# segasai/rvspecfit

Measured on AMD Instinct MI355X. Metric: spectra/sec (CCF+chi2 grid) DESI 3-arm, higher is better.
Workload: dtype f64

## Files before the change

### rvspecfit_amd/csrc/ccf_fft.hip

```cpp
#include "common.h"

#define XC_NT 512
#define XC_NTW(n2) ((n2) >> 3)

struct XcLds {
  int t1;
  int c0;
  int t1c;
  int ca;
  size_t bytes;
};
#define XW_NT1C 73
#define XC_LDS_MAX (159 * 1024)
__host__ __device__ constexpr XcLds xc_lds_pair(int n2, int nlag) {
  const int t1 = n2, c0 = t1 + XC_NTW(n2);
  return {t1, c0, 0, 0, sizeof(double2) * (size_t)c0 + sizeof(double) * 2 * (size_t)nlag};
}
__host__ __device__ constexpr XcLds xc_lds_ws(int n2, int nlag, bool ratio) {
  const int t1 = 2 * n2, c0 = t1 + XC_NTW(n2), t1c = c0 + ((nlag + 1) >> 1),
            ca = t1c + XW_NT1C;
  return {t1, c0, t1c, ca,
          sizeof(double2) * (size_t)ca + (ratio ? sizeof(double) * (size_t)nlag : 0)};
}
__host__ __device__ constexpr XcLds xc_lds_ws2(int n2, int nlag) {
  const int t1 = 4 * n2, c0 = t1 + XC_NTW(n2);
  return {t1, c0, 0, 0, sizeof(double2) * (size_t)c0 + sizeof(double) * 2 * (size_t)nlag};
}
__host__ __device__ constexpr bool xc_lds_fits(const XcLds &L, int n2, int nimg,
                                               int nrow, int nlag, bool ws, bool ratio) {
  const size_t D2 = sizeof(double2), D = sizeof(double);
  size_t end = D2 * (size_t)nimg * n2;
  if (D2 * L.t1 < end) return false;
  end = D2 * (L.t1 + XC_NTW(n2));
  if (D2 * L.c0 < end) return false;
  end = D2 * L.c0 + D * (size_t)nrow * nlag;
  if (ws) {
    if (D2 * L.t1c < end) return false;
    end = D2 * (L.t1c + 72);
    if (D2 * L.ca < end) return false;
    end = D2 * L.ca + (ratio ? D * (size_t)nlag : 0);
  }
  return end <= L.bytes && L.bytes <= XC_LDS_MAX;
}
constexpr bool xc_lds_check() {
  for (int nlag = 2; nlag <= 512; nlag++)
    for (int n2 = 2048; n2 <= 4096; n2 *= 2) {
      for (int ratio = 0; ratio < 2; ratio++)
        if (!xc_lds_fits(xc_lds_ws(n2, nlag, ratio), n2, 2, 1, nlag, true, ratio))
          return false;
      if (n2 == 2048 && !xc_lds_fits(xc_lds_ws2(n2, nlag), n2, 4, 2, nlag, false, false))
        return false;
      if (!xc_lds_fits(xc_lds_pair(n2, nlag), n2, 1, 2, nlag, false, false))
        return false;
    }
  return true;
}
static_assert(xc_lds_check(), "an LDS array of a cross-correlation kernel overlaps "
                              "its neighbour or ends beyond the launch's request");

__device__ __forceinline__ double2 cmul(double2 a, double2 b) {
  return make_double2(a.x * b.x - a.y * b.y, a.x * b.y + a.y * b.x);
}
__device__ __forceinline__ double2 cadd(double2 a, double2 b) {
  return make_double2(a.x + b.x, a.y + b.y);
}
__device__ __forceinline__ double2 csub(double2 a, double2 b) {
  return make_double2(a.x - b.x, a.y - b.y);
}
template <int SIGN>
__device__ __forceinline__ double2 cmuli(double2 a) {
  return (SIGN > 0) ? make_double2(-a.y, a.x) : make_double2(a.y, -a.x);
}

__host__ __device__ inline int xc_plan(int log2n, int *rad) {
  int n = 0, l = log2n;
  while (l >= 3) {
    rad[n++] = 8;
    l -= 3;
  }
  if (l == 2) rad[n++] = 4;
  if (l == 1) rad[n++] = 2;
  return n;
}

extern "C" int rvs_ccf_fft_pos(int nfft, int f) {
  int log2n = 0;
  while ((2 << log2n) < nfft) log2n++;
  int rad[8];
  const int np = xc_plan(log2n, rad);
  int n2 = nfft >> 1, pos = 0, m = n2;
  for (int p = 0; p < np; p++) {
    const int q = f % rad[p];
    f /= rad[p];
    m /= rad[p];
    pos += q * m;
  }
  return pos;
}

template <int SIGN>
__device__ __forceinline__ void dft4(double2 &a0, double2 &a1, double2 &a2,
                                     double2 &a3) {
  const double2 t0 = cadd(a0, a2), t1 = csub(a0, a2);
  const double2 t2 = cadd(a1, a3), t3 = cmuli<SIGN>(csub(a1, a3));
  a0 = cadd(t0, t2);
  a2 = csub(t0, t2);
  a1 = cadd(t1, t3);
  a3 = csub(t1, t3);
}

template <int SIGN>
__device__ __forceinline__ void dft8(double2 *a) {
  double2 e0 = a[0], e1 = a[2], e2 = a[4], e3 = a[6];
  double2 o0 = a[1], o1 = a[3], o2 = a[5], o3 = a[7];
  dft4<SIGN>(e0, e1, e2, e3);
  dft4<SIGN>(o0, o1, o2, o3);
  const double h = 0.70710678118654752440;
  const double2 w1o = (SIGN > 0) ? make_double2(h * (o1.x - o1.y), h * (o1.x + o1.y))
                                 : make_double2(h * (o1.x + o1.y), h * (o1.y - o1.x));
  const double2 w2o = cmuli<SIGN>(o2);
  const double2 w3o = (SIGN > 0) ? make_double2(-h * (o3.x + o3.y), h * (o3.x - o3.y))
                                 : make_double2(h * (o3.y - o3.x), -h * (o3.x + o3.y));
  a[0] = cadd(e0, o0);
  a[4] = csub(e0, o0);
  a[1] = cadd(e1, w1o);
  a[5] = csub(e1, w1o);
  a[2] = cadd(e2, w2o);
  a[6] = csub(e2, w2o);
  a[3] = cadd(e3, w3o);
  a[7] = csub(e3, w3o);
}

template <int SIGN>
__device__ __forceinline__ double2 twid(const double2 *__restrict__ tw, int e,
                                        int nfft) {
  const int half = nfft >> 1;
  double2 w = (e < half) ? tw[e] : tw[e - half];
  if (e >= half) {
    w.x = -w.x;
    w.y = -w.y;
  }
  if (SIGN < 0) w.y = -w.y;
  return w;
}

#ifdef RVS_XC_TIMING
__device__ unsigned long long xc_dbg[16];
#define XC_T(i)                                        \
  do {                                                 \
    __syncthreads();                                   \
    if (threadIdx.x == 0) {                            \
      const unsigned long long t_ = wall_clock64();    \
      atomicAdd(&xc_dbg[i], t_ - t_prev);              \
      t_prev = t_;                                     \
    }                                                  \
  } while (0)
extern "C" int rvs_dbg_read_xc(unsigned long long *out) {
  return hipMemcpyFromSymbol(out, HIP_SYMBOL(xc_dbg), sizeof(xc_dbg)) ==
                 hipSuccess
             ? 0
             : -1;
}
#else
#define XC_T(i)
#endif

template <int NT>
__device__ __forceinline__ void xc_fill_twiddles(double2 *a, int n2,
                                                 const double2 *__restrict__ tw) {
  const int ntw = XC_NTW(n2);
  if ((ntw & 63) == 0) {
    const int lane = threadIdx.x & 63;
    for (int i0 = (threadIdx.x >> 6) * 64; i0 < ntw; i0 += NT) {
      __builtin_amdgcn_global_load_lds(
          (const __attribute__((address_space(1))) void *)(tw + 2 * (i0 + lane)),
          (__attribute__((address_space(3))) void *)(a + n2 + i0), 16, 0, 0);
    }
    return;
  }
  for (int i = threadIdx.x; i < ntw; i += NT) a[n2 + i] = tw[2 * i];
}

struct XcMasks {
  unsigned g, b0, b7;
};
template <int NT>
__device__ __forceinline__ XcMasks xc_load_masks(const uint8_t *__restrict__ prune,
                                                 int n2) {
  XcMasks m = {0u, 0u, 0u};
  if (prune && (n2 >> 3) <= NT) {
    const int t = threadIdx.x, B = t >> 3;
    if (t < (n2 >> 3)) m.g = prune[(n2 >> 6) + t];
    if (B < (n2 >> 6)) {
      m.b0 = prune[(n2 >> 6) + 8 * B];
      m.b7 = prune[(n2 >> 6) + 8 * B + 7];
    }
  }
  return m;
}

template <int SIGN, int NT>
__device__ void fft_lds(double2 *a, int log2n, const double2 *__restrict__ tw,
                        const uint8_t *__restrict__ prune = nullptr,
                        const XcMasks *pm = nullptr) {
  const int n2 = 1 << log2n, nfft = n2 << 1;
  const double2 *T1 = a + n2;
  auto tw1 = [&](int r, int tws) -> double2 {
    double2 w = T1[r << (tws - 1)];
    if (SIGN < 0) w.y = -w.y;
    return w;
  };
  int rad[8];
  const int np = xc_plan(log2n, rad);
  const bool pr = prune && np >= 2 && rad[np - 1] == 8 && rad[np - 2] == 8;
  bool fold = false;
  const bool can_fold = pr && pm && (n2 >> 3) <= NT;
  int lgM = log2n;
  for (int p = 0; p < np; p++) {
    if (can_fold && p == 0) {
      const int pos8 = threadIdx.x & 7;
      const unsigned m = pm->g;
      const bool bad =
          m != 0 && !((pos8 == 0 && m == 0x01u) || (pos8 == 7 && m == 0x80u));
      fold = !__syncthreads_or(bad);
    }
    if (fold && p == np - 2) {
      __syncthreads();
      const int s = threadIdx.x & 7;
      for (int B = threadIdx.x >> 3; B < (n2 >> 6); B += NT >> 3) {
        const unsigned m0 = pm->b0 & 1u, m63 = pm->b7 >> 7;
        if (!(m0 | m63)) continue;
        double2 v[8];
#pragma unroll
        for (int j = 0; j < 8; j++) v[j] = a[B * 64 + s + 8 * j];
        dft8<SIGN>(v);
        double2 w = T1[s << (log2n - 6)];
        if (SIGN > 0) w.y = -w.y;
        double2 x63 = cmul(v[7], w), x0 = v[0];
        auto sum8 = [](double x) {
          x += dpp_get<0xb1, 0xf, 0xf>(x);
          x += dpp_get<0x4e, 0xf, 0xf>(x);
          x += dpp_get<0x141, 0xf, 0xf>(x);
          return x;
        };
        if (m0) {
          x0.x = sum8(x0.x);
          x0.y = sum8(x0.y);
          if (s == 0) a[B * 64] = x0;
        }
        if (m63) {
          x63.x = sum8(x63.x);
          x63.y = sum8(x63.y);
          if (s == 0) a[B * 64 + 63] = x63;
        }
      }
      break;
    }
    const int R = rad[p], lgR = (R == 8) ? 3 : (R == 4 ? 2 : 1);
    const int lgMp = lgM - lgR, Mp = 1 << lgMp;
    const int tws = log2n + 1 - lgM;
    if (!(can_fold && p == 0)) __syncthreads();
    for (int u = threadIdx.x; u < (n2 >> lgR); u += NT) {
      const int blk = u >> lgMp, r = u & (Mp - 1);
      const int base = (blk << lgM) + r;
      if (pr && p == np - 2) {
        const unsigned mask = prune[blk];
        if (mask == 0) continue;
        double2 v[8];
#pragma unroll
        for (int j = 0; j < 8; j++) v[j] = a[base + Mp * j];
        dft8<SIGN>(v);
        double2 wp[8];
        wp[0] = make_double2(1.0, 0.0);
        wp[1] = tw1(r, tws);
        wp[2] = cmul(wp[1], wp[1]);
        wp[3] = cmul(wp[2], wp[1]);
        wp[4] = cmul(wp[2], wp[2]);
        wp[7] = cmul(wp[4], wp[3]);
        wp[5] = cmul(wp[4], wp[1]);
        wp[6] = cmul(wp[4], wp[2]);
#pragma unroll
        for (int q = 0; q < 8; q++)
          if (mask & (1u << q))
            a[base + Mp * q] = (q == 0) ? v[0] : cmul(v[q], wp[q]);
        continue;
      }
      if (pr && p == np - 1) {
        const unsigned mask = prune[(n2 >> 6) + u];
        if (mask == 0) continue;
        double2 v[8];
#pragma unroll
        for (int j = 0; j < 8; j++) v[j] = a[base + j];
        dft8<SIGN>(v);
#pragma unroll
        for (int q = 0; q < 8; q++)
          if (mask & (1u << q)) a[base + q] = v[q];
        continue;
      }
      if (R == 8) {
        double2 v[8];
#pragma unroll
        for (int j = 0; j < 8; j++) v[j] = a[base + Mp * j];
        dft8<SIGN>(v);
        if (Mp > 1) {
          const double2 w1 = tw1(r, tws);
          v[1] = cmul(v[1], w1);
          const double2 w2 = cmul(w1, w1);
          v[2] = cmul(v[2], w2);
          double2 wc = cmul(w2, w1);
          v[3] = cmul(v[3], wc);
          const double2 w4 = cmul(w2, w2);
          v[4] = cmul(v[4], w4);
          v[7] = cmul(v[7], cmul(w4, wc));
          wc = cmul(w4, w1);
          v[5] = cmul(v[5], wc);
          v[6] = cmul(v[6], cmul(w4, w2));
        }
#pragma unroll
        for (int q = 0; q < 8; q++) a[base + Mp * q] = v[q];
      } else if (R == 4) {
        double2 v0 = a[base], v1 = a[base + Mp],
                v2 = a[base + 2 * Mp], v3 = a[base + 3 * Mp];
        dft4<SIGN>(v0, v1, v2, v3);
        if (Mp > 1) {
          const double2 w1 = twid<SIGN>(tw, r << tws, nfft);
          const double2 w2 = cmul(w1, w1), w3 = cmul(w2, w1);
          v1 = cmul(v1, w1);
          v2 = cmul(v2, w2);
          v3 = cmul(v3, w3);
        }
        a[base] = v0;
        a[base + Mp] = v1;
        a[base + 2 * Mp] = v2;
        a[base + 3 * Mp] = v3;
      } else {
        const double2 v0 = a[base], v1 = a[base + Mp];
        double2 d = csub(v0, v1);
        if (Mp > 1) d = cmul(d, twid<SIGN>(tw, r << tws, nfft));
        a[base] = cadd(v0, v1);
        a[base + Mp] = d;
      }
    }
    lgM = lgMp;
  }
  __syncthreads();
}

__device__ __forceinline__ int fft_pos(int f, int log2n) {
  int pos = 0, lgm = log2n;
  while (lgm > 0) {
    const int lgr = lgm >= 3 ? 3 : lgm;
    lgm -= lgr;
    pos += (f & ((1 << lgr) - 1)) << lgm;
    f >>= lgr;
  }
  return pos;
}

template <bool MODEL>
__global__ void __launch_bounds__(XC_NT)
    ccf_rfft_kernel(const double *__restrict__ proc_spec,
                    const double *__restrict__ proc_ivar, int nfft, int log2n,
                    const double2 *__restrict__ tw, double2 *__restrict__ work,
                    double2 *__restrict__ work2) {
  extern __shared__ double2 fa[];
  const int b = blockIdx.x, which = blockIdx.y, tid = threadIdx.x;
  const int n2 = nfft >> 1;
  const double *ps = proc_spec + (int64_t)b * nfft;
  const double *pi = MODEL ? nullptr : proc_ivar + (int64_t)b * nfft;
  xc_fill_twiddles<XC_NT>(fa, n2, tw);
  for (int n = tid; n < n2; n += XC_NT) {
    double x0, x1;
    if (MODEL) {
      x0 = ps[2 * n];
      x1 = ps[2 * n + 1];
      if (which) {
        x0 *= x0;
        x1 *= x1;
      }
    } else if (which == 0) {
      x0 = ps[2 * n] * pi[2 * n];
      x1 = ps[2 * n + 1] * pi[2 * n + 1];
    } else {
      x0 = pi[2 * n];
      x1 = pi[2 * n + 1];
    }
    fa[n] = make_double2(x0, x1);
  }
  fft_lds<-1, XC_NT>(fa, log2n, tw);
  double2 *out = MODEL ? (which ? work2 : work) + (int64_t)b * (n2 + 1)
                       : work + ((int64_t)b * 2 + which) * (n2 + 1);
  for (int k = tid; k <= n2; k += XC_NT) {
    double2 X;
    if (k == 0 || k == n2) {
      const double2 z0 = fa[0];
      X = make_double2(k == 0 ? z0.x + z0.y : z0.x - z0.y, 0.0);
    } else {
      const double2 zk = fa[fft_pos(k, log2n)];
      const double2 zm = fa[fft_pos(n2 - k, log2n)];
      const double2 e = make_double2(zk.x + zm.x, zk.y - zm.y);
      const double2 d = make_double2(zk.x - zm.x, zk.y + zm.y);
      const double2 q = cmul(twid<-1>(tw, k, nfft), d);
      X = make_double2(0.5 * (e.x + q.y), 0.5 * (e.y - q.x));
    }
    out[k] = MODEL ? X : make_double2(X.x, -X.y);
  }
}

int ccf_model_rfft(const double *model, int nfft, int M, const double *twid,
                   double *fft, double *fft2, hipStream_t st) {
  int log2n = 0;
  while ((2 << log2n) < nfft) log2n++;
  if ((2 << log2n) != nfft || nfft < 64 || nfft > 16384 || M < 1) return RVS_E_ARG;
  static bool attr_set = false;
  if (!attr_set) {
    (void)hipFuncSetAttribute((const void *)ccf_rfft_kernel<true>,
                              hipFuncAttributeMaxDynamicSharedMemorySize, XC_LDS_MAX);
    (void)hipGetLastError();
    attr_set = true;
  }
  for (int b0 = 0; b0 < M; b0 += 65535) {
    const int nb = (M - b0 < 65535) ? (M - b0) : 65535;
    const int64_t o = (int64_t)b0 * ((nfft >> 1) + 1);
    hipLaunchKernelGGL(ccf_rfft_kernel<true>, dim3(nb, 2), dim3(XC_NT),
                       xc_lds_pair(nfft >> 1, 0).bytes, st,
                       model + (int64_t)b0 * nfft, (const double *)nullptr, nfft, log2n,
                       reinterpret_cast<const double2 *>(twid),
                       reinterpret_cast<double2 *>(fft) + o,
                       reinterpret_cast<double2 *>(fft2) + o);
    RVS_LAUNCH_CHECK();
  }
  return 0;
}

#define XB_NT 512

__device__ __forceinline__ bool xc_job(unsigned bid, int T, int B, int G, int &b,
                                       int &t) {
  const int xcd = bid & 7;
  const int slot = bid >> 3;
  const int tt = slot % G;
  const int q = slot / G;
  b = q % B;
  const int g = q / B;
  t = xcd + 8 * (g * G + tt);
  return t < T;
}
__host__ inline int64_t xc_nblocks(int T, int B, int G) {
  const int ntx = (T + 7) >> 3;
  const int ngrp = (ntx + G - 1) / G;
  return 8ll * ngrp * G * B;
}
__host__ inline int xc_group(int T, int nfft) {
  const int64_t per_t = 2ll * ((nfft >> 1) + 1) * 16;
  if (per_t * T <= (16ll << 20)) return 0;
#ifndef XC_GROUP_BYTES
#define XC_GROUP_BYTES (2ll << 20)
#endif
  int G = (int)(XC_GROUP_BYTES / per_t);
  const int ntx = (T + 7) >> 3;
  if (G < 1) G = 1;
  if (G > ntx) G = ntx;
  return G;
}

__global__ void __launch_bounds__(XB_NT)
    __attribute__((amdgpu_waves_per_eu(4, 4)))
    ccf_xcorr_kernel(const double2 *__restrict__ work, int nfft, int log2n,
                     const double2 *__restrict__ tfft,
                     const double2 *__restrict__ tfft2, int T,
                     const double2 *__restrict__ tw, int continuum,
                     const int32_t *__restrict__ lag_pos,
                     const double *__restrict__ lag_vel, int nlag,
                     const int32_t *__restrict__ ilo,
                     const double *__restrict__ vgrid, int nvel, double beta,
                     const uint8_t *__restrict__ prune,
                     double *__restrict__ chisq, int B, int G) {
  extern __shared__ double2 fa[];
  const int n2 = nfft >> 1, npair = n2 >> 1;
  double *c0 = reinterpret_cast<double *>(fa + xc_lds_pair(n2, nlag).c0);
  double *c1 = c0 + nlag;
  int t = blockIdx.x, b = blockIdx.y;
  if (G > 0 && !xc_job(blockIdx.x, T, B, G, b, t)) return;
  const int tid = threadIdx.x;
  const double2 *Sc = work + ((int64_t)b * 2) * (n2 + 1);
  const double2 *Vc = Sc + (n2 + 1);
  const double2 *F = tfft + (int64_t)t * (n2 + 1);
  const double2 *F2 = tfft2 + (int64_t)t * (n2 + 1);
  const double inv_n = 1.0 / nfft;
  const int npass = continuum ? 1 : 2;
  xc_fill_twiddles<XB_NT>(fa, n2, tw);
  XcMasks pmask = xc_load_masks<XB_NT>(prune, n2);
#ifdef RVS_XC_TIMING
  unsigned long long t_prev = wall_clock64();
#endif
  double *out = chisq + ((int64_t)b * T + t) * nvel;
  const bool pre = (nlag <= XB_NT) && (nvel <= XB_NT);
  int pre_pos = 0, pre_lo = 0;
  double pre_x0 = 0, pre_x1 = 1, pre_xg = 0, pre_old = 0;
  if (pre) {
    const int tv = min(tid, nvel - 1);
    pre_pos = lag_pos[min(tid, nlag - 1)];
    pre_lo = ilo[tv];
    pre_xg = vgrid[tv];
    pre_old = out[tv];
  }
  for (int pass = 0; pass < npass; pass++) {
    if (continuum) {
      typedef int v4i_t __attribute__((ext_vector_type(4)));
      const int nbytes = (n2 + 1) * 16;
      const __amdgpu_buffer_rsrc_t rF = __builtin_amdgcn_make_buffer_rsrc(
          (void *)F, 0, nbytes, 0x00020000);
      const __amdgpu_buffer_rsrc_t rF2 = __builtin_amdgcn_make_buffer_rsrc(
          (void *)F2, 0, nbytes, 0x00020000);
      const __amdgpu_buffer_rsrc_t rS = __builtin_amdgcn_make_buffer_rsrc(
          (void *)Sc, 0, nbytes, 0x00020000);
      const __amdgpu_buffer_rsrc_t rV = __builtin_amdgcn_make_buffer_rsrc(
          (void *)Vc, 0, nbytes, 0x00020000);
      const __amdgpu_buffer_rsrc_t rT = __builtin_amdgcn_make_buffer_rsrc(
          (void *)tw, 0, (npair + 1) * 16, 0x00020000);
      auto ld = [](const __amdgpu_buffer_rsrc_t &r, int off) {
        const v4i_t v = __builtin_amdgcn_raw_buffer_load_b128(r, off, 0, 0);
        return make_double2(__hiloint2double(v.y, v.x),
                            __hiloint2double(v.w, v.z));
      };
      if (tid == 0) {
        const double2 p1 = cmul(F[0], Sc[0]), p2 = cmul(F2[0], Vc[0]);
        const double2 q1 = cmul(F[n2], Sc[n2]), q2 = cmul(F2[n2], Vc[n2]);
        const double xk = p2.x - 2 * p1.x, xm = q2.x - 2 * q1.x;
        fa[0] = make_double2(xk + xm, xk - xm);
      }
      for (int k0 = 1 + tid; k0 <= npair; k0 += 2 * XB_NT) {
        double2 op[2][9];
        bool live[2];
#pragma unroll
        for (int u = 0; u < 2; u++) {
          const int kk = k0 + u * XB_NT;
          live[u] = kk <= npair;
          const int k = live[u] ? kk : k0;
          const int ok = k * 16, om = (n2 - k) * 16;
          op[u][0] = ld(rF, ok), op[u][1] = ld(rS, ok);
          op[u][2] = ld(rF2, ok), op[u][3] = ld(rV, ok);
          op[u][4] = ld(rF, om), op[u][5] = ld(rS, om);
          op[u][6] = ld(rF2, om), op[u][7] = ld(rV, om);
          op[u][8] = ld(rT, ok);
        }
#pragma unroll
        for (int u = 0; u < 2; u++) {
          const int k = k0 + u * XB_NT, m = n2 - k;
          const double2 p1 = cmul(op[u][0], op[u][1]),
                        p2 = cmul(op[u][2], op[u][3]);
          const double2 Xk = make_double2(p2.x - 2 * p1.x, p2.y - 2 * p1.y);
          const double2 q1 = cmul(op[u][4], op[u][5]),
                        q2 = cmul(op[u][6], op[u][7]);
          const double2 Xm = make_double2(q2.x - 2 * q1.x, q2.y - 2 * q1.y);
          const double2 e = make_double2(Xk.x + Xm.x, Xk.y - Xm.y);
          const double2 d = make_double2(Xk.x - Xm.x, Xk.y + Xm.y);
          const double2 q = cmul(op[u][8], d);
          if (live[u]) {
            fa[k] = make_double2(e.x - q.y, e.y + q.x);
            if (m != k) fa[m] = make_double2(e.x + q.y, -e.y + q.x);
          }
        }
      }
    } else
    for (int k = tid; k <= npair; k += XB_NT) {
      const int m = n2 - k;
      double2 Xk, Xm;
      if (continuum) {
        const double2 p1 = cmul(F[k], Sc[k]), p2 = cmul(F2[k], Vc[k]);
        Xk = make_double2(p2.x - 2 * p1.x, p2.y - 2 * p1.y);
        const double2 q1 = cmul(F[m], Sc[m]), q2 = cmul(F2[m], Vc[m]);
        Xm = make_double2(q2.x - 2 * q1.x, q2.y - 2 * q1.y);
      } else if (pass == 0) {
        Xk = cmul(F[k], Sc[k]);
        Xm = cmul(F[m], Sc[m]);
      } else {
        Xk = cmul(F2[k], Vc[k]);
        Xm = cmul(F2[m], Vc[m]);
      }
      if (k == 0) {
        fa[0] = make_double2(Xk.x + Xm.x, Xk.x - Xm.x);
      } else {
        const double2 e = make_double2(Xk.x + Xm.x, Xk.y - Xm.y);
        const double2 d = make_double2(Xk.x - Xm.x, Xk.y + Xm.y);
        const double2 q = cmul(tw[k], d);
        fa[k] = make_double2(e.x - q.y, e.y + q.x);
        if (m != k) fa[m] = make_double2(e.x + q.y, -e.y + q.x);
      }
    }
    if (pass == 0 && pre) {
      asm volatile("" : "+v"(pre_pos), "+v"(pre_lo));
      asm volatile("" : "+v"(pmask.g), "+v"(pmask.b0), "+v"(pmask.b7));
      pre_x0 = lag_vel[pre_lo];
      pre_x1 = lag_vel[pre_lo + 1];
    }
    XC_T(0);
    fft_lds<1, XB_NT>(fa, log2n, tw, prune, &pmask);
    XC_T(1);
    const double *fr = reinterpret_cast<const double *>(fa);
    double *dst = (pass == 0) ? c0 : c1;
    if (pre) {
      if (tid < nlag) dst[tid] = fr[pre_pos] * inv_n;
    } else {
      for (int l = tid; l < nlag; l += XB_NT) dst[l] = fr[lag_pos[l]] * inv_n;
    }
    __syncthreads();
  }
  if (!continuum) {
    for (int l = tid; l < nlag; l += XB_NT) c0[l] = -c0[l] * c0[l] / c1[l];
    __syncthreads();
  }
  if (pre) {
    if (tid < nvel) {
      const double sl = (c0[pre_lo + 1] - c0[pre_lo]) / (pre_x1 - pre_x0);
      const double val = sl * (pre_xg - pre_x0) + c0[pre_lo];
      out[tid] = (beta != 0.0) ? beta * pre_old + val : val;
    }
    XC_T(2);
    return;
  }
  for (int v = tid; v < nvel; v += XB_NT) {
    const int lo = ilo[v];
    const double x0 = lag_vel[lo], x1 = lag_vel[lo + 1];
    const double sl = (c0[lo + 1] - c0[lo]) / (x1 - x0);
    const double val = sl * (vgrid[v] - x0) + c0[lo];
    out[v] = (beta != 0.0) ? beta * out[v] + val : val;
  }
}


#define XW_NT 1024
#define XW_HALF 512

template <int SIGN, int LOG2N>
__device__ __forceinline__ void xw_pass(double2 *a, const double2 *T1, int p, int t,
                                        const double2 *Tc = nullptr) {
  const int lgM = LOG2N - 3 * p, lgMp = lgM - 3, Mp = 1 << lgMp;
  const int tws = LOG2N + 1 - lgM;
  const int blk = t >> lgMp, r = t & (Mp - 1);
  const int base = (blk << lgM) + r;
  double2 v[8];
#pragma unroll
  for (int j = 0; j < 8; j++) v[j] = a[base + Mp * j];
  dft8<SIGN>(v);
  if (Mp > 1) {
    double2 w1 = Tc ? Tc[r] : T1[r << (tws - 1)];
    if (SIGN < 0) w1.y = -w1.y;
    v[1] = cmul(v[1], w1);
    const double2 w2 = cmul(w1, w1);
    v[2] = cmul(v[2], w2);
    double2 wc = cmul(w2, w1);
    v[3] = cmul(v[3], wc);
    const double2 w4 = cmul(w2, w2);
    v[4] = cmul(v[4], w4);
    v[7] = cmul(v[7], cmul(w4, wc));
    wc = cmul(w4, w1);
    v[5] = cmul(v[5], wc);
    v[6] = cmul(v[6], cmul(w4, w2));
  }
#pragma unroll
  for (int q = 0; q < 8; q++) a[base + Mp * q] = v[q];
}

template <int LOG2N, bool RATIO>
__global__ void __launch_bounds__(XW_NT)
    ccf_xcorr_ws_kernel(const double2 *__restrict__ work,
                        const double2 *__restrict__ tfft,
                        const double2 *__restrict__ tfft2, int T,
                        const double2 *__restrict__ tw,
                        const int32_t *__restrict__ lag_pos,
                        const double *__restrict__ lag_vel, int nlag,
                        const int32_t *__restrict__ ilo,
                        const double *__restrict__ vgrid, int nvel, double beta,
                        const uint8_t *__restrict__ prune,
                        double *__restrict__ chisq) {
  extern __shared__ double2 fa[];
  constexpr int log2n = LOG2N, n2 = 1 << LOG2N, nfft = 2 * n2, npair = n2 / 2;
  constexpr int NPP = npair / XW_HALF;
  constexpr bool P12 = (LOG2N == 12);
  static_assert(LOG2N == 12 || LOG2N == 11, "plans 8,8,8,8 and 8,8,8,4 only");
  auto img = [&](int i) -> double2 * { return fa + (i & 1) * n2; };
  const XcLds lds = xc_lds_ws(n2, nlag, RATIO);
  const double2 *T1 = fa + lds.t1;
  double *c0 = reinterpret_cast<double *>(fa + lds.c0);
  double2 *T1c = fa + lds.t1c;
  double *cA = reinterpret_cast<double *>(fa + lds.ca);
  const int TI = RATIO ? 2 * T : T;
  const int b = blockIdx.x, tid = threadIdx.x;
  const bool producer = tid >= XW_HALF;
  const int pt = tid & (XW_HALF - 1);
  const double inv_n = 1.0 / nfft;
  if (P12 && tid < 72)
    T1c[tid] = tid < 64 ? tw[2 * (tid << 3)] : tw[2 * ((tid - 64) << (log2n - 6))];
  xc_fill_twiddles<XW_NT>(fa + n2, n2, tw);
  XcMasks pmask = {0u, 0u, 0u};
  bool bad = !P12;
  if (P12 && !producer) {
    pmask = xc_load_masks<XW_HALF>(prune, n2);
    const int pos8 = pt & 7;
    const unsigned m = pmask.g;
    bad = m != 0 && !((pos8 == 0 && m == 0x01u) || (pos8 == 7 && m == 0x80u));
  }
  const bool fold = !__syncthreads_or(bad);
  const double2 *Sc = work + ((int64_t)b * 2) * (n2 + 1);
  const double2 *Vc = Sc + (n2 + 1);
  typedef int v4i_t __attribute__((ext_vector_type(4)));
  auto ld = [](const __amdgpu_buffer_rsrc_t &r, int off) {
    const v4i_t v = __builtin_amdgcn_raw_buffer_load_b128(r, off, 0, 0);
    return make_double2(__hiloint2double(v.y, v.x), __hiloint2double(v.w, v.z));
  };
  const int nbytes = (n2 + 1) * 16;
  if (producer) {
    double2 Sk[NPP], Vk[NPP], Sm[NPP], Vm[NPP];
#pragma unroll
    for (int u = 0; u < NPP; u++) {
      const int k = 1 + pt + u * XW_HALF, m = n2 - k;
      Sk[u] = Sc[k], Vk[u] = Vc[k], Sm[u] = Sc[m], Vm[u] = Vc[m];
    }
    const __amdgpu_buffer_rsrc_t rT = __builtin_amdgcn_make_buffer_rsrc(
        (void *)tw, 0, (npair + 1) * 16, 0x00020000);
    double2 op[2][5];
    auto issue = [&](int t, int u, double2 *o) {
      const int tt = RATIO ? (t >> 1) : t;
      const __amdgpu_buffer_rsrc_t rF = __builtin_amdgcn_make_buffer_rsrc(
          (void *)(((RATIO && (t & 1)) ? tfft2 : tfft) + (int64_t)tt * (n2 + 1)), 0,
          nbytes, 0x00020000);
      const __amdgpu_buffer_rsrc_t rF2 = __builtin_amdgcn_make_buffer_rsrc(
          (void *)(tfft2 + (int64_t)tt * (n2 + 1)), 0, nbytes, 0x00020000);
      int ptv = pt;
      asm volatile("" : "+v"(ptv));
      const int k = 1 + ptv + u * XW_HALF;
      const int ok = k * 16, om = (n2 - k) * 16;
      if (RATIO) {
        o[0] = ld(rF, ok);
        o[2] = ld(rF, om);
      } else {
        o[0] = ld(rF, ok), o[1] = ld(rF2, ok);
        o[2] = ld(rF, om), o[3] = ld(rF2, om);
      }
      o[4] = ld(rT, ok);
    };
    double2 dc[4];
    auto form = [&](double2 *dst, int u, const double2 *o, int tcur) {
      int ptv = pt;
      asm volatile("" : "+v"(ptv));
      const int k = 1 + ptv + u * XW_HALF, m = n2 - k;
      double2 Xk, Xm;
      if (RATIO) {
        const bool second = (tcur & 1) != 0;
        Xk = cmul(o[0], second ? Vk[u] : Sk[u]);
        Xm = cmul(o[2], second ? Vm[u] : Sm[u]);
      } else {
        const double2 p1 = cmul(o[0], Sk[u]), p2 = cmul(o[1], Vk[u]);
        Xk = make_double2(p2.x - 2 * p1.x, p2.y - 2 * p1.y);
        const double2 q1 = cmul(o[2], Sm[u]), q2 = cmul(o[3], Vm[u]);
        Xm = make_double2(q2.x - 2 * q1.x, q2.y - 2 * q1.y);
      }
      const double2 e = make_double2(Xk.x + Xm.x, Xk.y - Xm.y);
      const double2 d = make_double2(Xk.x - Xm.x, Xk.y + Xm.y);
      const double2 q = cmul(o[4], d);
      dst[k] = make_double2(e.x - q.y, e.y + q.x);
      if (m != k) dst[m] = make_double2(e.x + q.y, -e.y + q.x);
      if (u == NPP - 1 && ptv == 0) {
        double xk, xm;
        if (RATIO) {
          const bool second = (tcur & 1) != 0;
          xk = cmul(second ? dc[1] : dc[0], second ? Vc[0] : Sc[0]).x;
          xm = cmul(second ? dc[3] : dc[2], second ? Vc[n2] : Sc[n2]).x;
        } else {
          const double2 a1 = cmul(dc[0], Sc[0]), a2 = cmul(dc[1], Vc[0]);
          const double2 b1 = cmul(dc[2], Sc[n2]), b2 = cmul(dc[3], Vc[n2]);
          xk = a2.x - 2 * a1.x, xm = b2.x - 2 * b1.x;
        }
        dst[0] = make_double2(xk + xm, xk - xm);
      }
    };
    const int nbar = (P12 && fold) ? 4 : 5;
    issue(0, 0, op[0]);
    if (NPP == 2) issue(0, 1, op[1]);
    for (int it = -1; it < TI; it++) {
      const int tn = it + 1;
      if (tn < TI) {
        double2 *dst = img(tn);
        {
          const int tt = RATIO ? (tn >> 1) : tn;
          const double2 *Fp = tfft + (int64_t)tt * (n2 + 1);
          const double2 *F2p = tfft2 + (int64_t)tt * (n2 + 1);
          dc[0] = Fp[0], dc[1] = F2p[0], dc[2] = Fp[n2], dc[3] = F2p[n2];
        }
        if (NPP == 2) {
#pragma unroll
          for (int u = 0; u < 2; u++) {
            form(dst, u, op[u], tn);
            if (tn + 1 < TI) issue(tn + 1, u, op[u]);
            __syncthreads();
          }
        } else {
#pragma unroll
          for (int u = 0; u < NPP; u++) {
            if (u + 1 < NPP)
              issue(tn, u + 1, op[(u + 1) & 1]);
            else if (tn + 1 < TI)
              issue(tn + 1, 0, op[(u + 1) & 1]);
            form(dst, u, op[u & 1], tn);
            __syncthreads();
          }
        }
        for (int q = NPP; q < nbar; q++) __syncthreads();
      } else {
        for (int q = 0; q < nbar; q++) __syncthreads();
      }
    }
    return;
  }
  const int tvx = min(pt, nvel - 1);
  const int pre_pos = lag_pos[min(pt, nlag - 1)];
  const int pre_lo = ilo[tvx];
  const double pre_xg = vgrid[tvx];
  const double pre_x0 = lag_vel[pre_lo], pre_x1 = lag_vel[pre_lo + 1];
  for (int it = -1; it < TI; it++) {
    if (it < 0) {
      const int nbar = (P12 && fold) ? 4 : 5;
      for (int q = 0; q < nbar; q++) __syncthreads();
      continue;
    }
    double2 *a = img(it);
    double *out = chisq + ((int64_t)b * T + (RATIO ? (it >> 1) : it)) * nvel;
    double pre_old = 0;
    if (beta != 0.0) pre_old = out[tvx];
    if (pt < (n2 >> 3)) xw_pass<1, LOG2N>(a, T1, 0, pt);
    __syncthreads();
    if (pt < (n2 >> 3)) xw_pass<1, LOG2N>(a, T1, 1, pt, P12 ? T1c : nullptr);
    __syncthreads();
    if (!P12) {
      if (pt < (n2 >> 3)) xw_pass<1, LOG2N>(a, T1, 2, pt);
      __syncthreads();
      {
        const int base = pt << 2;
        double2 v0 = a[base], v1 = a[base + 1], v2 = a[base + 2], v3 = a[base + 3];
        dft4<1>(v0, v1, v2, v3);
        a[base] = v0, a[base + 1] = v1, a[base + 2] = v2, a[base + 3] = v3;
      }
      __syncthreads();
    } else if (fold) {
      const int s = pt & 7;
      const int B = pt >> 3;
      const unsigned m0 = pmask.b0 & 1u, m63 = pmask.b7 >> 7;
      if (m0 | m63) {
        double2 v[8];
#pragma unroll
        for (int j = 0; j < 8; j++) v[j] = a[B * 64 + s + 8 * j];
        dft8<1>(v);
        double2 w = T1c[64 + s];
        w.y = -w.y;
        double2 x63 = cmul(v[7], w), x0 = v[0];
        auto sum8 = [](double x) {
          x += dpp_get<0xb1, 0xf, 0xf>(x);
          x += dpp_get<0x4e, 0xf, 0xf>(x);
          x += dpp_get<0x141, 0xf, 0xf>(x);
          return x;
        };
        if (m0) {
          x0.x = sum8(x0.x);
          x0.y = sum8(x0.y);
          if (s == 0) a[B * 64] = x0;
        }
        if (m63) {
          x63.x = sum8(x63.x);
          x63.y = sum8(x63.y);
          if (s == 0) a[B * 64 + 63] = x63;
        }
      }
      __syncthreads();
    } else {
      {
        const int blk = pt >> 3, r = pt & 7, base = (blk << 6) + r;
        const unsigned mask = prune[blk];
        if (mask != 0) {
          double2 v[8];
#pragma unroll
          for (int j = 0; j < 8; j++) v[j] = a[base + 8 * j];
          dft8<1>(v);
          double2 wp[8];
          wp[0] = make_double2(1.0, 0.0);
          wp[1] = T1[r << (log2n + 1 - 6 - 1)];
          wp[2] = cmul(wp[1], wp[1]);
          wp[3] = cmul(wp[2], wp[1]);
          wp[4] = cmul(wp[2], wp[2]);
          wp[7] = cmul(wp[4], wp[3]);
          wp[5] = cmul(wp[4], wp[1]);
          wp[6] = cmul(wp[4], wp[2]);
#pragma unroll
          for (int q = 0; q < 8; q++)
            if (mask & (1u << q))
              a[base + 8 * q] = (q == 0) ? v[0] : cmul(v[q], wp[q]);
        }
      }
      __syncthreads();
      {
        const unsigned mask = pmask.g;
        if (mask != 0) {
          const int base = pt << 3;
          double2 v[8];
#pragma unroll
          for (int j = 0; j < 8; j++) v[j] = a[base + j];
          dft8<1>(v);
#pragma unroll
          for (int q = 0; q < 8; q++)
            if (mask & (1u << q)) a[base + q] = v[q];
        }
      }
      __syncthreads();
    }
    if (RATIO) {
      if (pt < nlag) {
        const double c = reinterpret_cast<const double *>(a)[pre_pos] * inv_n;
        if (it & 1)
          c0[pt] = -cA[pt] * cA[pt] / c;
        else
          cA[pt] = c;
      }
    } else if (pt < nlag) {
      c0[pt] = reinterpret_cast<const double *>(a)[pre_pos] * inv_n;
    }
    __syncthreads();
    if ((!RATIO || (it & 1)) && pt < nvel) {
      const double sl = (c0[pre_lo + 1] - c0[pre_lo]) / (pre_x1 - pre_x0);
      const double val = sl * (pre_xg - pre_x0) + c0[pre_lo];
      out[pt] = (beta != 0.0) ? beta * pre_old + val : val;
    }
  }
}

__global__ void __launch_bounds__(XW_NT)
    ccf_xcorr_ws2_kernel(const double2 *__restrict__ work,
                         const double2 *__restrict__ tfft,
                         const double2 *__restrict__ tfft2, int T,
                         const double2 *__restrict__ tw,
                         const int32_t *__restrict__ lag_pos,
                         const double *__restrict__ lag_vel, int nlag,
                         const int32_t *__restrict__ ilo,
                         const double *__restrict__ vgrid, int nvel, double beta,
                         double *__restrict__ chisq) {
  extern __shared__ double2 fa[];
  constexpr int LOG2N = 11, n2 = 1 << LOG2N, nfft = 2 * n2, npair = n2 / 2;
  constexpr int NBAR = 5;
  auto img = [&](int i, int j) -> double2 * { return fa + (((i & 1) << 1) + j) * n2; };
  const XcLds lds = xc_lds_ws2(n2, nlag);
  const double2 *T1 = fa + lds.t1;
  double *c0 = reinterpret_cast<double *>(fa + lds.c0);
  const int b = blockIdx.x, tid = threadIdx.x;
  const bool producer = tid >= XW_HALF;
  const int pt = tid & (XW_HALF - 1);
  const double inv_n = 1.0 / nfft;
  xc_fill_twiddles<XW_NT>(fa + 3 * n2, n2, tw);
  const double2 *Sc = work + ((int64_t)b * 2) * (n2 + 1);
  const double2 *Vc = Sc + (n2 + 1);
  typedef int v4i_t __attribute__((ext_vector_type(4)));
  auto ld = [](const __amdgpu_buffer_rsrc_t &r, int off) {
    const v4i_t v = __builtin_amdgcn_raw_buffer_load_b128(r, off, 0, 0);
    return make_double2(__hiloint2double(v.y, v.x), __hiloint2double(v.w, v.z));
  };
  const int nbytes = (n2 + 1) * 16;
  const int NIT = (T + 1) >> 1;
  __syncthreads();
  if (producer) {
    double2 Sk[2], Vk[2], Sm[2], Vm[2];
#pragma unroll
    for (int u = 0; u < 2; u++) {
      const int k = 1 + pt + u * XW_HALF, m = n2 - k;
      Sk[u] = Sc[k], Vk[u] = Vc[k], Sm[u] = Sc[m], Vm[u] = Vc[m];
    }
    const __amdgpu_buffer_rsrc_t rT = __builtin_amdgcn_make_buffer_rsrc(
        (void *)tw, 0, (npair + 1) * 16, 0x00020000);
    double2 op[2][5];
    auto issue = [&](int t, int u, double2 *o) {
      const __amdgpu_buffer_rsrc_t rF = __builtin_amdgcn_make_buffer_rsrc(
          (void *)(tfft + (int64_t)t * (n2 + 1)), 0, nbytes, 0x00020000);
      const __amdgpu_buffer_rsrc_t rF2 = __builtin_amdgcn_make_buffer_rsrc(
          (void *)(tfft2 + (int64_t)t * (n2 + 1)), 0, nbytes, 0x00020000);
      const int k = 1 + pt + u * XW_HALF;
      const int ok = k * 16, om = (n2 - k) * 16;
      o[0] = ld(rF, ok), o[1] = ld(rF2, ok);
      o[2] = ld(rF, om), o[3] = ld(rF2, om);
      o[4] = ld(rT, ok);
    };
    auto form = [&](double2 *dst, int t, int u, const double2 *o) {
      const int k = 1 + pt + u * XW_HALF, m = n2 - k;
      const double2 p1 = cmul(o[0], Sk[u]), p2 = cmul(o[1], Vk[u]);
      const double2 Xk = make_double2(p2.x - 2 * p1.x, p2.y - 2 * p1.y);
      const double2 q1 = cmul(o[2], Sm[u]), q2 = cmul(o[3], Vm[u]);
      const double2 Xm = make_double2(q2.x - 2 * q1.x, q2.y - 2 * q1.y);
      const double2 e = make_double2(Xk.x + Xm.x, Xk.y - Xm.y);
      const double2 d = make_double2(Xk.x - Xm.x, Xk.y + Xm.y);
      const double2 q = cmul(o[4], d);
      dst[k] = make_double2(e.x - q.y, e.y + q.x);
      if (m != k) dst[m] = make_double2(e.x + q.y, -e.y + q.x);
      if (u == 1 && pt == 0) {
        const double2 *Fp = tfft + (int64_t)t * (n2 + 1);
        const double2 *F2p = tfft2 + (int64_t)t * (n2 + 1);
        const double2 a1 = cmul(Fp[0], Sc[0]), a2 = cmul(F2p[0], Vc[0]);
        const double2 b1 = cmul(Fp[n2], Sc[n2]), b2 = cmul(F2p[n2], Vc[n2]);
        const double xk = a2.x - 2 * a1.x, xm = b2.x - 2 * b1.x;
        dst[0] = make_double2(xk + xm, xk - xm);
      }
    };
    auto tq = [&](int i, int q) { return min(2 * i + (q >> 1), T - 1); };
    issue(tq(0, 0), 0, op[0]);
    for (int it = -1; it < NIT; it++) {
      const int in = it + 1;
      if (in < NIT) {
#pragma unroll
        for (int q = 0; q < 4; q++) {
          if (q + 1 < 4)
            issue(tq(in, q + 1), (q + 1) & 1, op[(q + 1) & 1]);
          else if (in + 1 < NIT)
            issue(tq(in + 1, 0), 0, op[(q + 1) & 1]);
          form(img(in, q >> 1), tq(in, q), q & 1, op[q & 1]);
          __syncthreads();
        }
        __syncthreads();
      } else {
        for (int q = 0; q < NBAR; q++) __syncthreads();
      }
    }
    return;
  }
  const int j = pt >> 8, bt = pt & 255;
  int pre_pos[1], dummy = 0;
  (void)dummy;
  pre_pos[0] = lag_pos[min(pt, nlag - 1)];
  const int tvx = min(pt, nvel - 1);
  const int pre_lo = ilo[tvx];
  const double pre_xg = vgrid[tvx];
  const double pre_x0 = lag_vel[pre_lo], pre_x1 = lag_vel[pre_lo + 1];
  for (int it = -1; it < NIT; it++) {
    if (it < 0) {
      for (int q = 0; q < NBAR; q++) __syncthreads();
      continue;
    }
    double2 *a = img(it, j);
    const int t0 = 2 * it, t1 = min(2 * it + 1, T - 1);
    const bool two = (2 * it + 1 < T);
    double *out0 = chisq + ((int64_t)b * T + t0) * nvel;
    double *out1 = chisq + ((int64_t)b * T + t1) * nvel;
    double old0 = 0, old1 = 0;
    if (beta != 0.0) {
      old0 = out0[tvx];
      old1 = out1[tvx];
    }
    xw_pass<1, LOG2N>(a, T1, 0, bt);
    __syncthreads();
    xw_pass<1, LOG2N>(a, T1, 1, bt);
    __syncthreads();
    xw_pass<1, LOG2N>(a, T1, 2, bt);
    __syncthreads();
#pragma unroll
    for (int h = 0; h < 2; h++) {
      const int base = (bt + 256 * h) << 2;
      double2 v0 = a[base], v1 = a[base + 1], v2 = a[base + 2], v3 = a[base + 3];
      dft4<1>(v0, v1, v2, v3);
      a[base] = v0, a[base + 1] = v1, a[base + 2] = v2, a[base + 3] = v3;
    }
    __syncthreads();
    if (pt < nlag) {
      c0[pt] = reinterpret_cast<const double *>(img(it, 0))[pre_pos[0]] * inv_n;
      c0[nlag + pt] = reinterpret_cast<const double *>(img(it, 1))[pre_pos[0]] * inv_n;
    }
    __syncthreads();
    if (pt < nvel) {
      const double dx = pre_x1 - pre_x0, xg = pre_xg - pre_x0;
      const double sl0 = (c0[pre_lo + 1] - c0[pre_lo]) / dx;
      const double val0 = sl0 * xg + c0[pre_lo];
      out0[pt] = (beta != 0.0) ? beta * old0 + val0 : val0;
      if (two) {
        const double sl1 = (c0[nlag + pre_lo + 1] - c0[nlag + pre_lo]) / dx;
        const double val1 = sl1 * xg + c0[nlag + pre_lo];
        out1[pt] = (beta != 0.0) ? beta * old1 + val1 : val1;
      }
    }
  }
}

extern "C" int rvs_ccf_xcorr(const double *proc_spec, const double *proc_ivar,
                             int nfft, int B, const double *tfft,
                             const double *tfft2, int T, const double *twid_,
                             int continuum, const int32_t *lag_pos,
                             const double *lag_vel, int nlag, const int32_t *ilo,
                             const double *vgrid, int nvel, double beta,
                             const uint8_t *prune, double *chisq, double *work,
                             void *stream) {
  int log2n = 0;
  while ((2 << log2n) < nfft) log2n++;
  if ((2 << log2n) != nfft || nfft < 64 || nfft > 16384) return RVS_E_ARG;
  if (B < 1 || T < 1 || T > 65535 || nlag < 2 || nvel < 1) return RVS_E_ARG;
  const int n2 = nfft >> 1;
  const size_t shm1 = xc_lds_pair(n2, 0).bytes;
  const size_t shm2 = xc_lds_pair(n2, nlag).bytes;
  if (shm2 > XC_LDS_MAX) return RVS_E_ARG;
  hipStream_t st = rvs_stream(stream);
  const double2 *tw = reinterpret_cast<const double2 *>(twid_);
  static bool attr_set = false;
  if (!attr_set) {
    (void)hipFuncSetAttribute((const void *)ccf_rfft_kernel<false>,
                              hipFuncAttributeMaxDynamicSharedMemorySize,
                              XC_LDS_MAX);
    (void)hipFuncSetAttribute((const void *)ccf_xcorr_kernel,
                              hipFuncAttributeMaxDynamicSharedMemorySize,
                              XC_LDS_MAX);
    (void)hipGetLastError();
    attr_set = true;
  }
  hipLaunchKernelGGL(ccf_rfft_kernel<false>, dim3(B, 2), dim3(XC_NT), shm1, st,
                     proc_spec, proc_ivar, nfft, log2n, tw,
                     reinterpret_cast<double2 *>(work), (double2 *)nullptr);
  RVS_LAUNCH_CHECK();
  const int G = xc_group(T, nfft);
  {
    const bool ws_on = rvs_opt(RVS_OPT_XC_WS) != 0;
    const bool p12 = (nfft == 8192 && prune), p11 = (nfft == 4096);
    if (ws_on && (p12 || p11) && nlag <= XW_HALF && nvel <= XW_HALF && T >= 2) {
      static bool ws_attr = false;
      if (!ws_attr) {
        (void)hipFuncSetAttribute((const void *)ccf_xcorr_ws_kernel<12, false>,
                                  hipFuncAttributeMaxDynamicSharedMemorySize,
                                  XC_LDS_MAX);
        (void)hipFuncSetAttribute((const void *)ccf_xcorr_ws_kernel<12, true>,
                                  hipFuncAttributeMaxDynamicSharedMemorySize,
                                  XC_LDS_MAX);
        (void)hipFuncSetAttribute((const void *)ccf_xcorr_ws_kernel<11, true>,
                                  hipFuncAttributeMaxDynamicSharedMemorySize,
                                  XC_LDS_MAX);
        (void)hipFuncSetAttribute((const void *)ccf_xcorr_ws2_kernel,
                                  hipFuncAttributeMaxDynamicSharedMemorySize,
                                  XC_LDS_MAX);
        (void)hipGetLastError();
        ws_attr = true;
      }
      const size_t shmw = xc_lds_ws(n2, nlag, !continuum).bytes;
#define RVS_XW_ARGS                                                                 \
  reinterpret_cast<const double2 *>(work), reinterpret_cast<const double2 *>(tfft),  \
      reinterpret_cast<const double2 *>(tfft2), T, tw, lag_pos, lag_vel, nlag, ilo,  \
      vgrid, nvel, beta, prune, chisq
      if (!continuum) {
        if (p12)
          hipLaunchKernelGGL((ccf_xcorr_ws_kernel<12, true>), dim3(B), dim3(XW_NT), shmw,
                             st, RVS_XW_ARGS);
        else
          hipLaunchKernelGGL((ccf_xcorr_ws_kernel<11, true>), dim3(B), dim3(XW_NT), shmw,
                             st, RVS_XW_ARGS);
        RVS_LAUNCH_CHECK();
        return 0;
      }
      if (p12)
        hipLaunchKernelGGL((ccf_xcorr_ws_kernel<12, false>), dim3(B), dim3(XW_NT), shmw, st,
                           reinterpret_cast<const double2 *>(work),
                           reinterpret_cast<const double2 *>(tfft),
                           reinterpret_cast<const double2 *>(tfft2), T, tw, lag_pos,
                           lag_vel, nlag, ilo, vgrid, nvel, beta, prune, chisq);
      else
        hipLaunchKernelGGL(ccf_xcorr_ws2_kernel, dim3(B), dim3(XW_NT),
                           xc_lds_ws2(n2, nlag).bytes, st,
                           reinterpret_cast<const double2 *>(work),
                           reinterpret_cast<const double2 *>(tfft),
                           reinterpret_cast<const double2 *>(tfft2), T, tw, lag_pos,
                           lag_vel, nlag, ilo, vgrid, nvel, beta, chisq);
      RVS_LAUNCH_CHECK();
      return 0;
    }
  }
  const int bmax = G ? (int)(0x7fffffffll / xc_nblocks(T, 1, G)) : 65535;
  for (int b0 = 0; b0 < B; b0 += bmax) {
    const int nb = (B - b0 < bmax) ? (B - b0) : bmax;
    const dim3 grid = G ? dim3((unsigned)xc_nblocks(T, nb, G)) : dim3(T, nb);
    hipLaunchKernelGGL(
        ccf_xcorr_kernel, grid, dim3(XB_NT), shm2, st,
        reinterpret_cast<const double2 *>(work) + (int64_t)b0 * 2 * (n2 + 1),
        nfft, log2n, reinterpret_cast<const double2 *>(tfft),
        reinterpret_cast<const double2 *>(tfft2), T, tw, continuum, lag_pos,
        lag_vel, nlag, ilo, vgrid, nvel, beta, prune,
        chisq + (int64_t)b0 * T * nvel, nb, G);
    RVS_LAUNCH_CHECK();
  }
  return 0;
}
```

Baseline: 76600.

## Scatter folded CCF lag values directly to c0 and cut block barriers

In the pruned 4096-point fold path, a small LDS lookup table now maps each block's first and last output element to its lag index, so the reduced values are written straight into c0/cA instead of back into the FFT image and then gathered. This removes the image write-back, the separate gather step and its barrier. A wave-level barrier replaces one block barrier after pass 1, and the producer half now syncs every second form step, so each iteration has two block barriers instead of four. The change adds LDS for the table and a one-time setup, and it relies on per-wave data ownership being correct for the wave barrier.

```diff
diff --git a/rvspecfit_amd/csrc/ccf_fft.hip b/rvspecfit_amd/csrc/ccf_fft.hip
--- a/rvspecfit_amd/csrc/ccf_fft.hip
+++ b/rvspecfit_amd/csrc/ccf_fft.hip
@@ -8,23 +8,27 @@
   int c0;
   int t1c;
   int ca;
+  int lt;
   size_t bytes;
 };
 #define XW_NT1C 73
+#define XW_NLT 256
 #define XC_LDS_MAX (159 * 1024)
 __host__ __device__ constexpr XcLds xc_lds_pair(int n2, int nlag) {
   const int t1 = n2, c0 = t1 + XC_NTW(n2);
-  return {t1, c0, 0, 0, sizeof(double2) * (size_t)c0 + sizeof(double) * 2 * (size_t)nlag};
+  return {t1, c0, 0, 0, 0,
+          sizeof(double2) * (size_t)c0 + sizeof(double) * 2 * (size_t)nlag};
 }
 __host__ __device__ constexpr XcLds xc_lds_ws(int n2, int nlag, bool ratio) {
   const int t1 = 2 * n2, c0 = t1 + XC_NTW(n2), t1c = c0 + ((nlag + 1) >> 1),
-            ca = t1c + XW_NT1C;
-  return {t1, c0, t1c, ca,
-          sizeof(double2) * (size_t)ca + (ratio ? sizeof(double) * (size_t)nlag : 0)};
+            ca = t1c + XW_NT1C, lt = ca + (ratio ? (nlag + 1) >> 1 : 0);
+  return {t1, c0, t1c, ca, lt,
+          sizeof(double2) * (size_t)lt + sizeof(int32_t) * (size_t)XW_NLT};
 }
 __host__ __device__ constexpr XcLds xc_lds_ws2(int n2, int nlag) {
   const int t1 = 4 * n2, c0 = t1 + XC_NTW(n2);
-  return {t1, c0, 0, 0, sizeof(double2) * (size_t)c0 + sizeof(double) * 2 * (size_t)nlag};
+  return {t1, c0, 0, 0, 0,
+          sizeof(double2) * (size_t)c0 + sizeof(double) * 2 * (size_t)nlag};
 }
 __host__ __device__ constexpr bool xc_lds_fits(const XcLds &L, int n2, int nimg,
                                                int nrow, int nlag, bool ws, bool ratio) {
@@ -39,6 +43,8 @@
     end = D2 * (L.t1c + 72);
     if (D2 * L.ca < end) return false;
     end = D2 * L.ca + (ratio ? D * (size_t)nlag : 0);
+    if (D2 * L.lt < end) return false;
+    end = D2 * L.lt + sizeof(int32_t) * (size_t)XW_NLT;
   }
   return end <= L.bytes && L.bytes <= XC_LDS_MAX;
 }
@@ -686,6 +692,7 @@
   double *c0 = reinterpret_cast<double *>(fa + lds.c0);
   double2 *T1c = fa + lds.t1c;
   double *cA = reinterpret_cast<double *>(fa + lds.ca);
+  int32_t *lt = reinterpret_cast<int32_t *>(fa + lds.lt);
   const int TI = RATIO ? 2 * T : T;
   const int b = blockIdx.x, tid = threadIdx.x;
   const bool producer = tid >= XW_HALF;
@@ -702,7 +709,15 @@
     const unsigned m = pmask.g;
     bad = m != 0 && !((pos8 == 0 && m == 0x01u) || (pos8 == 7 && m == 0x80u));
   }
+  if (P12 && tid < XW_NLT) lt[tid] = -1;
   const bool fold = !__syncthreads_or(bad);
+  if (P12) {
+    if (fold && tid < nlag) {
+      const int p = lag_pos[tid], e = (p >> 1) & 63;
+      if (e == 0 || e == 63) lt[(((p >> 7) & 63) << 2) + (e ? 2 : 0) + (p & 1)] = tid;
+    }
+    __syncthreads();
+  }
   const double2 *Sc = work + ((int64_t)b * 2) * (n2 + 1);
   const double2 *Vc = Sc + (n2 + 1);
   typedef int v4i_t __attribute__((ext_vector_type(4)));
@@ -776,7 +791,8 @@
         dst[0] = make_double2(xk + xm, xk - xm);
       }
     };
-    const int nbar = (P12 && fold) ? 4 : 5;
+    const bool two = P12 && fold;
+    const int nbar = two ? 2 : 5;
     issue(0, 0, op[0]);
     if (NPP == 2) issue(0, 1, op[1]);
     for (int it = -1; it < TI; it++) {
@@ -804,10 +820,10 @@
             else if (tn + 1 < TI)
               issue(tn + 1, 0, op[(u + 1) & 1]);
             form(dst, u, op[u & 1], tn);
-            __syncthreads();
+            if (!two || (u & 1)) __syncthreads();
           }
         }
-        for (int q = NPP; q < nbar; q++) __syncthreads();
+        for (int q = two ? NPP / 2 : NPP; q < nbar; q++) __syncthreads();
       } else {
         for (int q = 0; q < nbar; q++) __syncthreads();
       }
@@ -819,9 +835,12 @@
   const int pre_lo = ilo[tvx];
   const double pre_xg = vgrid[tvx];
   const double pre_x0 = lag_vel[pre_lo], pre_x1 = lag_vel[pre_lo + 1];
+  typedef int v4i32_t __attribute__((ext_vector_type(4)));
+  v4i32_t lag = {-1, -1, -1, -1};
+  if (P12) lag = reinterpret_cast<const v4i32_t *>(lt)[pt >> 3];
   for (int it = -1; it < TI; it++) {
     if (it < 0) {
-      const int nbar = (P12 && fold) ? 4 : 5;
+      const int nbar = (P12 && fold) ? 2 : 5;
       for (int q = 0; q < nbar; q++) __syncthreads();
       continue;
     }
@@ -832,18 +851,10 @@
     if (pt < (n2 >> 3)) xw_pass<1, LOG2N>(a, T1, 0, pt);
     __syncthreads();
     if (pt < (n2 >> 3)) xw_pass<1, LOG2N>(a, T1, 1, pt, P12 ? T1c : nullptr);
-    __syncthreads();
-    if (!P12) {
-      if (pt < (n2 >> 3)) xw_pass<1, LOG2N>(a, T1, 2, pt);
-      __syncthreads();
-      {
-        const int base = pt << 2;
-        double2 v0 = a[base], v1 = a[base + 1], v2 = a[base + 2], v3 = a[base + 3];
-        dft4<1>(v0, v1, v2, v3);
-        a[base] = v0, a[base + 1] = v1, a[base + 2] = v2, a[base + 3] = v3;
-      }
-      __syncthreads();
-    } else if (fold) {
+    if (P12 && fold) {
+      __builtin_amdgcn_fence(__ATOMIC_RELEASE, "wavefront");
+      __builtin_amdgcn_wave_barrier();
+      __builtin_amdgcn_fence(__ATOMIC_ACQUIRE, "wavefront");
       const int s = pt & 7;
       const int B = pt >> 3;
       const unsigned m0 = pmask.b0 & 1u, m63 = pmask.b7 >> 7;
@@ -861,70 +872,93 @@
           x += dpp_get<0x141, 0xf, 0xf>(x);
           return x;
         };
+        auto put = [&](int l, double x) {
+          if (l < 0) return;
+          const double c = x * inv_n;
+          if (!RATIO)
+            c0[l] = c;
+          else if (it & 1)
+            c0[l] = -cA[l] * cA[l] / c;
+          else
+            cA[l] = c;
+        };
         if (m0) {
           x0.x = sum8(x0.x);
           x0.y = sum8(x0.y);
-          if (s == 0) a[B * 64] = x0;
+          if (s == 0) put(lag.x, x0.x), put(lag.y, x0.y);
         }
         if (m63) {
           x63.x = sum8(x63.x);
           x63.y = sum8(x63.y);
-          if (s == 0) a[B * 64 + 63] = x63;
+          if (s == 0) put(lag.z, x63.x), put(lag.w, x63.y);
         }
       }
       __syncthreads();
     } else {
-      {
-        const int blk = pt >> 3, r = pt & 7, base = (blk << 6) + r;
-        const unsigned mask = prune[blk];
-        if (mask != 0) {
-          double2 v[8];
-#pragma unroll
-          for (int j = 0; j < 8; j++) v[j] = a[base + 8 * j];
-          dft8<1>(v);
-          double2 wp[8];
-          wp[0] = make_double2(1.0, 0.0);
-          wp[1] = T1[r << (log2n + 1 - 6 - 1)];
-          wp[2] = cmul(wp[1], wp[1]);
-          wp[3] = cmul(wp[2], wp[1]);
-          wp[4] = cmul(wp[2], wp[2]);
-          wp[7] = cmul(wp[4], wp[3]);
-          wp[5] = cmul(wp[4], wp[1]);
-          wp[6] = cmul(wp[4], wp[2]);
-#pragma unroll
-          for (int q = 0; q < 8; q++)
-            if (mask & (1u << q))
-              a[base + 8 * q] = (q == 0) ? v[0] : cmul(v[q], wp[q]);
-        }
-      }
       __syncthreads();
-      {
-        const unsigned mask = pmask.g;
-        if (mask != 0) {
-          const int base = pt << 3;
-          double2 v[8];
-#pragma unroll
-          for (int j = 0; j < 8; j++) v[j] = a[base + j];
-          dft8<1>(v);
-#pragma unroll
-          for (int q = 0; q < 8; q++)
-            if (mask & (1u << q)) a[base + q] = v[q];
-        }
+      if (!P12) {
+        if (pt < (n2 >> 3)) xw_pass<1, LOG2N>(a, T1, 2, pt);
+        __syncthreads();
+        {
+          const int base = pt << 2;
+          double2 v0 = a[base], v1 = a[base + 1], v2 = a[base + 2], v3 = a[base + 3];
+          dft4<1>(v0, v1, v2, v3);
+          a[base] = v0, a[base + 1] = v1, a[base + 2] = v2, a[base + 3] = v3;
+        }
+        __syncthreads();
+      } else {
+        {
+          const int blk = pt >> 3, r = pt & 7, base = (blk << 6) + r;
+          const unsigned mask = prune[blk];
+          if (mask != 0) {
+            double2 v[8];
+  #pragma unroll
+            for (int j = 0; j < 8; j++) v[j] = a[base + 8 * j];
+            dft8<1>(v);
+            double2 wp[8];
+            wp[0] = make_double2(1.0, 0.0);
+            wp[1] = T1[r << (log2n + 1 - 6 - 1)];
+            wp[2] = cmul(wp[1], wp[1]);
+            wp[3] = cmul(wp[2], wp[1]);
+            wp[4] = cmul(wp[2], wp[2]);
+            wp[7] = cmul(wp[4], wp[3]);
+            wp[5] = cmul(wp[4], wp[1]);
+            wp[6] = cmul(wp[4], wp[2]);
+  #pragma unroll
+            for (int q = 0; q < 8; q++)
+              if (mask & (1u << q))
+                a[base + 8 * q] = (q == 0) ? v[0] : cmul(v[q], wp[q]);
+          }
+        }
+        __syncthreads();
+        {
+          const unsigned mask = pmask.g;
+          if (mask != 0) {
+            const int base = pt << 3;
+            double2 v[8];
+  #pragma unroll
+            for (int j = 0; j < 8; j++) v[j] = a[base + j];
+            dft8<1>(v);
+  #pragma unroll
+            for (int q = 0; q < 8; q++)
+              if (mask & (1u << q)) a[base + q] = v[q];
+          }
+        }
+        __syncthreads();
+      }
+      if (RATIO) {
+        if (pt < nlag) {
+          const double c = reinterpret_cast<const double *>(a)[pre_pos] * inv_n;
+          if (it & 1)
+            c0[pt] = -cA[pt] * cA[pt] / c;
+          else
+            cA[pt] = c;
+        }
+      } else if (pt < nlag) {
+        c0[pt] = reinterpret_cast<const double *>(a)[pre_pos] * inv_n;
       }
       __syncthreads();
     }
-    if (RATIO) {
-      if (pt < nlag) {
-        const double c = reinterpret_cast<const double *>(a)[pre_pos] * inv_n;
-        if (it & 1)
-          c0[pt] = -cA[pt] * cA[pt] / c;
-        else
-          cA[pt] = c;
-      }
-    } else if (pt < nlag) {
-      c0[pt] = reinterpret_cast<const double *>(a)[pre_pos] * inv_n;
-    }
-    __syncthreads();
     if ((!RATIO || (it & 1)) && pt < nvel) {
       const double sl = (c0[pre_lo + 1] - c0[pre_lo]) / (pre_x1 - pre_x0);
       const double val = sl * (pre_xg - pre_x0) + c0[pre_lo];
```

Result: faster. 78030 (median of 6 runs) (+1.9%).
